# lambdaclass/simpleworks

Measured on AMD Instinct MI355X. Metric: Marlin prove() constraints/sec at 2^20 R1CS; G1 MSM points/sec, higher is better.
Workload: dtype u32 limbs (384-bit Montgomery Fq for G1, 256-bit Fr); 1 GPU; marlin_prove: synthetic R1CS, 2^20 constraints = variables = non-zeros per matrix (|H| = |K| = 2^20), SRS + proving key device resident; per_gpu_units=1048576, multi_gpu=replicas (one proof per rank)

## Files before the change

include/swmarlin.h:

```cpp
#ifndef SWMARLIN_H
#define SWMARLIN_H
#include <stddef.h>
#include <stdint.h>
#ifdef __cplusplus
extern "C" {
#endif

#define SWM_OK 0
#define SWM_ERR_INVALID_ARG (-1)
#define SWM_ERR_NO_DEVICE (-2)
#define SWM_ERR_HIP (-3)
#define SWM_ERR_OOM (-4)
#define SWM_ERR_UNSATISFIED (-5)
#define SWM_ERR_INDEX_TOO_LARGE (-6)
#define SWM_ERR_SERIALIZATION (-7)
#define SWM_ERR_MISMATCH (-8)
#define SWM_ERR_INTERNAL (-9)

typedef struct swm_ctx swm_ctx;
typedef struct swm_bases swm_bases;

int swm_version(void);
const char *swm_strerror(int code);
int swm_init(int device, swm_ctx **out);
void swm_destroy(swm_ctx *ctx);
const char *swm_last_error(swm_ctx *ctx);
int swm_set_stream(swm_ctx *ctx, void *hip_stream);
int swm_synchronize(swm_ctx *ctx);
int swm_malloc(swm_ctx *ctx, size_t bytes, void **dptr);
int swm_free(swm_ctx *ctx, void *dptr);
int swm_memcpy_h2d(swm_ctx *ctx, void *dst_dev, const void *src_host, size_t bytes);
int swm_memcpy_d2h(swm_ctx *ctx, void *dst_host, const void *src_dev, size_t bytes);

int swm_srs_upload(swm_ctx *ctx, const uint64_t *xy, size_t n, swm_bases **out);
int swm_srs_free(swm_ctx *ctx, swm_bases *bases);
size_t swm_srs_len(const swm_bases *bases);
int swm_msm_g1(swm_ctx *ctx, const swm_bases *bases, size_t offset, const uint64_t *scalars, size_t n,
               uint64_t out_jac[18]);
int swm_msm_g1_dev(swm_ctx *ctx, const swm_bases *bases, size_t offset, const void *d_scalars, size_t n,
                   int scalars_montgomery, uint64_t out_jac[18]);
int swm_g1_normalize(const uint64_t jac[18], uint64_t out_xy[12], int *is_inf);
int swm_g1_add_jac(const uint64_t a[18], const uint64_t b[18], uint64_t out[18]);

int swm_ntt_fr(swm_ctx *ctx, uint64_t *data, unsigned log_n, int inverse, int coset);
int swm_ntt_fr_dev(swm_ctx *ctx, void *d_data, unsigned log_n, int inverse, int coset);
int swm_ntt_fr_sharded_dev(swm_ctx *ctx, void *d_local, unsigned log_n, int inverse, int blocks_in);

int swm_spmv_fr(swm_ctx *ctx, const uint32_t *rowptr, const uint32_t *col, const uint64_t *val, const uint64_t *z,
                size_t z_len, uint64_t *out, size_t rows, size_t nnz);
int swm_spmv_fr_dev(swm_ctx *ctx, const void *d_rowptr, const void *d_col, const void *d_val, const void *d_z,
                    void *d_out, size_t rows);

int swm_batch_inverse_fr(swm_ctx *ctx, uint64_t *data, size_t n);
int swm_batch_inverse_fr_dev(swm_ctx *ctx, void *d_data, size_t n);
int swm_vec_mul_fr(swm_ctx *ctx, const uint64_t *a, const uint64_t *b, uint64_t *out, size_t n);
int swm_vec_mul_fr_dev(swm_ctx *ctx, const void *d_a, const void *d_b, void *d_out, size_t n);

typedef struct swm_rng swm_rng;
typedef struct swm_srs swm_srs;
typedef struct swm_pk swm_pk;
typedef struct swm_vk swm_vk;

int swm_rng_test_new(swm_rng **out);
int swm_rng_from_seed(const uint8_t seed[32], swm_rng **out);
typedef void (*swm_fill_bytes_fn)(void *user, uint8_t *dest, size_t len);
int swm_rng_from_callback(swm_fill_bytes_fn fill_bytes, void *user, swm_rng **out);
int swm_rng_from_chacha(const uint8_t key[32], uint64_t word_pos, int rounds, swm_rng **out);
int swm_rng_word_pos(const swm_rng *rng, uint64_t *word_pos);
int swm_rng_fill_bytes(swm_rng *rng, uint8_t *dest, size_t len);
void swm_rng_fill_bytes_cb(void *user, uint8_t *dest, size_t len);
void swm_rng_free(swm_rng *rng);
int swm_rng_next_u64(swm_rng *rng, uint64_t *out);
int swm_rng_rand_fr(swm_rng *rng, uint64_t out_mont[4]);

typedef struct swm_r1cs {
    size_t num_instance, num_witness, num_constraints;
    const uint64_t *instance;
    const uint64_t *witness;
    const uint32_t *a_rowptr, *a_col; const uint64_t *a_val;
    const uint32_t *b_rowptr, *b_col; const uint64_t *b_val;
// ... 369 lines not shown
```

simpleworks_amd/_lib.py:

```python
import contextlib
import ctypes
import json
import os

import numpy as np

_HERE = os.path.dirname(os.path.abspath(__file__))
LIB_PATH = os.environ.get("SWM_LIB_PATH") or os.path.join(_HERE, "libswmarlin.so")

_u64p = ctypes.POINTER(ctypes.c_uint64)
_u32p = ctypes.POINTER(ctypes.c_uint32)
_vp = ctypes.c_void_p
_sz = ctypes.c_size_t
_int = ctypes.c_int

ABI = {
    "swm_version": (_int, []),
    "swm_strerror": (ctypes.c_char_p, [_int]),
    "swm_init": (_int, [_int, ctypes.POINTER(_vp)]),
    "swm_destroy": (None, [_vp]),
    "swm_last_error": (ctypes.c_char_p, [_vp]),
    "swm_set_stream": (_int, [_vp, _vp]),
    "swm_set_msm_sharding": (_int, [_vp, ctypes.c_uint, ctypes.c_uint, _vp, _vp]),
    "swm_rccl_unique_id": (_int, [ctypes.c_void_p]),
    "swm_rccl_init": (_int, [_vp, ctypes.c_void_p, ctypes.c_uint, ctypes.c_uint]),
    "swm_set_rccl_comm": (_int, [_vp, _vp, ctypes.c_uint, ctypes.c_uint]),
    "swm_selftest_exchange": (_int, [_vp, ctypes.c_void_p, ctypes.c_void_p, _sz, _int]),
    "swm_rccl_info": (_int, [ctypes.c_char_p, _sz]),
    "swm_exchange_stats": (_int, [_vp, ctypes.POINTER(ctypes.c_uint64), ctypes.POINTER(ctypes.c_uint64)]),
    "swm_synchronize": (_int, [_vp]),
    "swm_malloc": (_int, [_vp, _sz, ctypes.POINTER(_vp)]),
    "swm_free": (_int, [_vp, _vp]),
    "swm_memcpy_h2d": (_int, [_vp, _vp, _vp, _sz]),
    "swm_memcpy_d2h": (_int, [_vp, _vp, _vp, _sz]),
    "swm_srs_upload": (_int, [_vp, _u64p, _sz, ctypes.POINTER(_vp)]),
    "swm_srs_free": (_int, [_vp, _vp]),
    "swm_srs_len": (_sz, [_vp]),
    "swm_msm_g1": (_int, [_vp, _vp, _sz, _u64p, _sz, _u64p]),
    "swm_msm_g1_dev": (_int, [_vp, _vp, _sz, _vp, _sz, _int, _u64p]),
    "swm_g1_normalize": (_int, [_u64p, _u64p, ctypes.POINTER(_int)]),
    "swm_g1_add_jac": (_int, [_u64p, _u64p, _u64p]),
    "swm_ntt_fr": (_int, [_vp, _u64p, ctypes.c_uint, _int, _int]),
    "swm_ntt_fr_dev": (_int, [_vp, _vp, ctypes.c_uint, _int, _int]),
    "swm_ntt_fr_sharded_dev": (_int, [_vp, ctypes.c_void_p, ctypes.c_uint, _int, _int]),
    "swm_spmv_fr": (_int, [_vp, _u32p, _u32p, _u64p, _u64p, _sz, _u64p, _sz, _sz]),
    "swm_spmv_fr_dev": (_int, [_vp, _vp, _vp, _vp, _vp, _vp, _sz]),
    "swm_batch_inverse_fr": (_int, [_vp, _u64p, _sz]),
    "swm_batch_inverse_fr_dev": (_int, [_vp, _vp, _sz]),
    "swm_vec_mul_fr": (_int, [_vp, _u64p, _u64p, _u64p, _sz]),
    "swm_vec_mul_fr_dev": (_int, [_vp, _vp, _vp, _vp, _sz]),
    "swm_rng_test_new": (_int, [ctypes.POINTER(_vp)]),
    "swm_rng_from_seed": (_int, [ctypes.c_void_p, ctypes.POINTER(_vp)]),
    "swm_rng_from_callback": (_int, [_vp, _vp, ctypes.POINTER(_vp)]),
    "swm_rng_from_chacha": (_int, [ctypes.c_void_p, ctypes.c_uint64, _int, ctypes.POINTER(_vp)]),
    "swm_rng_word_pos": (_int, [_vp, ctypes.POINTER(ctypes.c_uint64)]),
    "swm_rng_fill_bytes": (_int, [_vp, ctypes.c_void_p, ctypes.c_size_t]),
    "swm_rng_fill_bytes_cb": (None, [_vp, ctypes.c_void_p, ctypes.c_size_t]),
    "swm_rng_free": (None, [_vp]),
    "swm_rng_next_u64": (_int, [_vp, ctypes.POINTER(ctypes.c_uint64)]),
    "swm_rng_rand_fr": (_int, [_vp, _u64p]),
    "swm_generate_universal_srs": (_int, [_vp, _sz, _sz, _sz, _vp, ctypes.POINTER(_vp)]),
    "swm_srs_destroy": (None, [_vp, _vp]),
    "swm_srs_max_degree": (_sz, [_vp]),
    "swm_srs_power_of_g": (_int, [_vp, _vp, _sz, _u64p]),
    "swm_srs_export": (_int, [_vp, _vp, _sz, _sz, _u64p, _u64p, _u64p, _u64p]),
    "swm_srs_import": (_int, [_vp, _u64p, _sz, _u64p, _u64p, _u64p, ctypes.POINTER(_vp)]),
    "swm_generate_proving_and_verifying_keys": (_int, [_vp, _vp, ctypes.c_void_p, ctypes.POINTER(_vp), ctypes.POINTER(_vp)]),
    "swm_pk_destroy": (None, [_vp, _vp]),
    "swm_pk_retain": (_int, [_vp]),
    "swm_pk_attach": (_int, [_vp, _vp]),
    "swm_pk_device": (_int, [_vp]),
    "swm_pk_refcount": (_int, [_vp]),
    "swm_device_mem_info": (_int, [_vp, ctypes.POINTER(_sz), ctypes.POINTER(_sz)]),
    "swm_vk_destroy": (None, [_vp]),
    "swm_generate_proof": (_int, [_vp, _vp, ctypes.c_void_p, _vp, ctypes.c_void_p, _sz, ctypes.POINTER(_sz)]),
# ... 268 lines not shown
        return self

    def download(self, shape, dtype=np.uint64):
        out = np.empty(shape, dtype=dtype)
        assert out.nbytes <= self.nbytes
        self.ctx._check(self.ctx.lib.swm_memcpy_d2h(self.ctx.h, out.ctypes.data, self.ptr, out.nbytes), "swm_memcpy_d2h")
        return out

    def free(self):
        if self.ptr:
            self.ctx.lib.swm_free(self.ctx.h, self.ptr)
            self.ptr = None


class Bases:
    def __init__(self, ctx, handle, n):
        self.ctx, self.h, self.n = ctx, handle, n

    def free(self):
        if self.h:
            self.ctx.lib.swm_srs_free(self.ctx.h, self.h)
            self.h = None


class Context:

    def __init__(self, device=0):
        self.lib = load_library()
        h = _vp()
        rc = self.lib.swm_init(device, ctypes.byref(h))
        if rc != 0:
            raise SwmError(rc, "swm_init")
        self.h = h
        self.device = device

    def close(self):
        if self.h:
            self.lib.swm_destroy(self.h)
            self.h = None

    def __del__(self):
        try:
            self.close()
        except Exception:
            pass

    def _check(self, rc, what):
        if rc != 0:
            raise SwmError(rc, what, self.lib.swm_last_error(self.h).decode(errors="replace"))

    def set_stream(self, stream_ptr):
        self._check(self.lib.swm_set_stream(self.h, stream_ptr), "swm_set_stream")

    def synchronize(self):
        self._check(self.lib.swm_synchronize(self.h), "swm_synchronize")

    def mem_info(self):
        free, total = ctypes.c_size_t(0), ctypes.c_size_t(0)
        self._check(self.lib.swm_device_mem_info(self.h, ctypes.byref(free), ctypes.byref(total)), "swm_device_mem_info")
        return free.value, total.value

    ALLGATHER_FN = ctypes.CFUNCTYPE(ctypes.c_int, ctypes.c_void_p, ctypes.c_void_p, ctypes.c_size_t, ctypes.c_void_p)

    def set_msm_sharding(self, rank, world, allgather=None):
        if world <= 1 or allgather is None:
            self._check(self.lib.swm_set_msm_sharding(self.h, 0, 1, None, None), "swm_set_msm_sharding")
            self._shard_cb = None
            self.shard_rank, self.shard_world = 0, 1
            return
        self.shard_rank, self.shard_world = rank, world

        def _cb(_user, send, nbytes, recv):
            try:
                out = allgather(ctypes.string_at(send, nbytes))
                if len(out) != nbytes * world:
                    return 1
                ctypes.memmove(recv, out, len(out))
                return 0
            except Exception:
                import traceback
                traceback.print_exc()
                return 1
        cb = Context.ALLGATHER_FN(_cb)
        self._check(self.lib.swm_set_msm_sharding(self.h, rank, world, ctypes.cast(cb, ctypes.c_void_p), None),
                    "swm_set_msm_sharding")
        self._shard_cb = cb

    def rccl_init(self, unique_id, rank, world):
        buf = (ctypes.c_uint8 * 128).from_buffer_copy(bytes(unique_id))
        self._check(self.lib.swm_rccl_init(self.h, buf, rank, world), "swm_rccl_init")

    def selftest_exchange(self, send_buf, recv_buf, bytes_per_peer, alltoall=True):
        self._check(self.lib.swm_selftest_exchange(self.h, send_buf.ptr, recv_buf.ptr, bytes_per_peer, int(alltoall)), "swm_selftest_exchange")

    def exchange_stats(self):
        calls, nbytes = ctypes.c_uint64(0), ctypes.c_uint64(0)
        self._check(self.lib.swm_exchange_stats(self.h, ctypes.byref(calls), ctypes.byref(nbytes)), "swm_exchange_stats")
        return calls.value, nbytes.value

    def alloc(self, nbytes):
        return DeviceBuffer(self, nbytes)

    def to_device(self, arr):
        arr = np.ascontiguousarray(arr)
        return DeviceBuffer(self, max(arr.nbytes, 64)).upload(arr)

# ... 902 lines not shown
```

simpleworks_amd/csrc/capi.hip:

```cpp
#include <dlfcn.h>
#include <stdarg.h>
#include <string.h>
#include <algorithm>
#include <vector>
#include "context.h"
#include "g1.cuh"
#include "msm.h"

struct swm_rccl_id_arg {
    char internal[128];
};

namespace swm {

int ntt_run(swm_ctx* ctx, void* d_data, unsigned log_n, int inverse, int coset);
int ntt_sharded_run(swm_ctx* ctx, void* d_local, unsigned log_n, int inverse, int blocks_in);
struct SpmvPlan;
int spmv_run(swm_ctx* ctx, const void* d_rowptr, const void* d_col, const void* d_val, const void* d_z, void* d_out,
             size_t rows, const SpmvPlan* plan = nullptr);
int vec_mul_run(swm_ctx* ctx, const void* a, const void* b, void* out, size_t n);
int batch_inverse_run(swm_ctx* ctx, void* d, size_t n);
int selftest_mul_run(swm_ctx* ctx, int which, const void* a, const void* b, void* out, size_t n);
int selftest_chain_run(swm_ctx* ctx, int which, void* out, size_t threads, int iters);
int selftest_g1_add_run(swm_ctx* ctx, const void* a, const void* b, void* out, size_t n);
// ... 466 lines not shown
    if (!rccl().ok) return rccl_unavailable(ctx);
    rccl_release(ctx);
    swm_rccl_id_arg arg;
    memcpy(arg.internal, id, 128);
    void* comm = nullptr;
    int rc = rccl().CommInitRank(&comm, (int)world, arg, (int)rank);
    if (rc != 0) return rccl_fail(ctx, "ncclCommInitRank", rc);
    ctx->rccl_comm = comm;
    ctx->rccl_own = true;
    ctx->shard_rank = rank;
    ctx->shard_world = world;
    ctx->shard_allgather = nullptr;
    ctx->shard_user = nullptr;
    return SWM_OK;
}
int swm_set_rccl_comm(swm_ctx* ctx, void* nccl_comm, unsigned rank, unsigned world) {
    if (!ctx) return SWM_ERR_INVALID_ARG;
    rccl_release(ctx);
    if (!nccl_comm) {
        ctx->shard_rank = 0;
        ctx->shard_world = 1;
        return SWM_OK;
    }
    if (world == 0 || rank >= world) return SWM_ERR_INVALID_ARG;
    if (!rccl().ok) return rccl_unavailable(ctx);
    ctx->rccl_comm = nccl_comm;
    ctx->rccl_own = false;
    ctx->shard_rank = rank;
    ctx->shard_world = world;
    ctx->shard_allgather = nullptr;
    ctx->shard_user = nullptr;
    return SWM_OK;
}
int swm_rccl_info(char* buf, size_t cap) {
    if (!buf || cap == 0) return SWM_ERR_INVALID_ARG;
    const std::string d = rccl_describe();
    snprintf(buf, cap, "%s", d.c_str());
    return rccl().ok ? SWM_OK : SWM_ERR_INTERNAL;
}
int swm_exchange_stats(swm_ctx* ctx, uint64_t* calls, uint64_t* bytes_per_rank) {
    if (!ctx) return SWM_ERR_INVALID_ARG;
    if (calls) *calls = ctx->stat_exchanges;
    if (bytes_per_rank) *bytes_per_rank = ctx->stat_exchange_bytes;
    return SWM_OK;
}

int swm_set_stream(swm_ctx* ctx, void* hip_stream) {
    if (!ctx) return SWM_ERR_INVALID_ARG;
    SWM_ON_DEVICE(ctx);
    SWM_HIP(ctx, hipStreamSynchronize(ctx->stream));
    ctx->stream = hip_stream ? (hipStream_t)hip_stream : ctx->own_stream;
    return SWM_OK;
}
int swm_synchronize(swm_ctx* ctx) {
    if (!ctx) return SWM_ERR_INVALID_ARG;
    SWM_ON_DEVICE(ctx);
    SWM_HIP(ctx, hipStreamSynchronize(ctx->stream));
    return SWM_OK;
}
int swm_malloc(swm_ctx* ctx, size_t bytes, void** dptr) {
    if (!ctx || !dptr) return SWM_ERR_INVALID_ARG;
    SWM_ON_DEVICE(ctx);
    SWM_HIP(ctx, hipMalloc(dptr, bytes ? bytes : 1));
    return SWM_OK;
}
int swm_free(swm_ctx* ctx, void* dptr) {
    if (!ctx) return SWM_ERR_INVALID_ARG;
    SWM_ON_DEVICE(ctx);
    SWM_HIP(ctx, hipStreamSynchronize(ctx->stream));
    SWM_HIP(ctx, hipFree(dptr));
    return SWM_OK;
}
int swm_memcpy_h2d(swm_ctx* ctx, void* dst, const void* src, size_t bytes) {
    if (!ctx) return SWM_ERR_INVALID_ARG;
    SWM_ON_DEVICE(ctx);
    SWM_HIP(ctx, hipMemcpyAsync(dst, src, bytes, hipMemcpyHostToDevice, ctx->stream));
    SWM_HIP(ctx, hipStreamSynchronize(ctx->stream));
    return SWM_OK;
}
int swm_memcpy_d2h(swm_ctx* ctx, void* dst, const void* src, size_t bytes) {
    if (!ctx) return SWM_ERR_INVALID_ARG;
    SWM_ON_DEVICE(ctx);
    SWM_HIP(ctx, hipMemcpyAsync(dst, src, bytes, hipMemcpyDeviceToHost, ctx->stream));
    SWM_HIP(ctx, hipStreamSynchronize(ctx->stream));
    return SWM_OK;
}

int swm_srs_upload(swm_ctx* ctx, const uint64_t* xy, size_t n, swm_bases** out) {
    if (!ctx || !xy || !out || n == 0) return set_err(ctx, SWM_ERR_INVALID_ARG, "srs_upload: bad arguments");
    SWM_ON_DEVICE(ctx);
    swm_bases* b = new swm_bases();
    b->n = n;
    hipError_t e = hipMalloc(&b->d_points, n * sizeof(G1Affine));
    if (e != hipSuccess) {
        delete b;
        return set_err(ctx, SWM_ERR_OOM, "srs_upload: %s", hipGetErrorString(e));
    }
    e = hipMemcpyAsync(b->d_points, xy, n * sizeof(G1Affine), hipMemcpyHostToDevice, ctx->stream);
    if (e == hipSuccess) e = hipStreamSynchronize(ctx->stream);
    if (e != hipSuccess) {
        (void)hipFree(b->d_points);
        delete b;
        return set_err(ctx, SWM_ERR_HIP, "srs_upload: %s", hipGetErrorString(e));
    }
    const size_t mask_words = (n + 31) / 32;
    int rc = SWM_OK;
// ... 436 lines not shown
```

simpleworks_amd/csrc/context.h:

```cpp
#pragma once
#include <hip/hip_runtime.h>
#include <stdint.h>
#include <stdio.h>
#include <map>
#include <string>
#include <vector>
#include "../../include/swmarlin.h"
#include "host/pool.h"
#include "host/witness_chunks.h"
#include "switches.h"

namespace swm {

struct MsmJob;
struct DevBuf {
    void* p = nullptr;
    size_t cap = 0;
};

struct NttTables {
    void* lo = nullptr;
    void* hi = nullptr;
    size_t hi_len = 0;
};
// ... 20 lines not shown
    size_t ntt_pass_table_bytes = 0;
    static constexpr int MSM_SLOTS = 8;
    static constexpr int MSM_LANES = 4;
    hipStream_t aux_stream[MSM_LANES] = {nullptr, nullptr, nullptr, nullptr};
    std::vector<hipStream_t> spare_streams;
    hipEvent_t fork_event = nullptr;
    void* pinned = nullptr;
    void* pinned_dev = nullptr;
    void* h2d_stage = nullptr;
    size_t h2d_stage_used = 0;
    const void* witness_dev = nullptr;
    size_t witness_stage_bytes = swm::WITNESS_STAGE_BYTES;
    hipEvent_t slot_event[MSM_SLOTS] = {nullptr};
    bool slot_busy[MSM_SLOTS] = {false};
    hipEvent_t acc_event[MSM_SLOTS] = {nullptr};
    hipEvent_t sort_event[MSM_SLOTS] = {nullptr};
    hipEvent_t set_acc_event[4] = {nullptr, nullptr, nullptr, nullptr};
    hipEvent_t lane_copy_event[4] = {nullptr, nullptr, nullptr, nullptr};
    hipEvent_t twin_sorted_event = nullptr;
    hipEvent_t twin_copy_event[MSM_SLOTS] = {nullptr};
    std::vector<swm::MsmJob*> pending_tails;
    swm::MsmJob* lazy_tail = nullptr;
    int next_slot = 0;
    std::multimap<size_t, void*> pool;
    uint64_t stat_msm_digits = 0;
    uint64_t stat_msm_twins = 0;
    uint64_t stat_msm_adds = 0;
    uint64_t stat_msm_zero_points = 0;
    uint64_t stat_spmv_nnz = 0;
    std::vector<std::pair<char, uint64_t>> call_log;
    void log_call(char kind, uint64_t v) {
        if (profiling && call_log.size() < 8192) call_log.push_back({kind, v});
    }
    uint64_t stat_msm_calls = 0, stat_msm_points = 0, stat_ntt_calls = 0, stat_ntt_elems = 0, stat_spmv_calls = 0,
             stat_spmv_rows = 0;
    int profiling = 0;
    bool prof_open = false;
    std::map<std::string, swm::ProfAgg> prof;
    std::vector<swm::ProfPending> pending;
    std::vector<hipEvent_t> event_pool;
    unsigned shard_rank = 0, shard_world = 1;
    swm_allgather_fn shard_allgather = nullptr;
    void* shard_user = nullptr;
    void* rccl_comm = nullptr;
    bool rccl_own = false;
    void *rccl_send = nullptr, *rccl_recv = nullptr;
    size_t rccl_cap = 0;
    uint64_t stat_exchanges = 0, stat_exchange_bytes = 0;
    swm::HostPool* host_pool = nullptr;
    hipStream_t copy_stream = nullptr;
    void* ext_pinned = nullptr;
    bool ext_registered = false;
    size_t msm_pipe_min = 0;
    size_t msm_slot_bytes[6] = {0, 0, 0, 0, 0, 0};
    bool emulated_exchange = false;
    unsigned msm_since_wait = 0;
    uint32_t* ext_totals = nullptr;
    hipEvent_t ext_cnt_event[8] = {nullptr, nullptr, nullptr, nullptr, nullptr, nullptr, nullptr, nullptr};
    hipEvent_t ext_event[5] = {nullptr, nullptr, nullptr, nullptr, nullptr};
};

struct swm_bases {
    void* d_points = nullptr;
    void* d_points28 = nullptr;
    uint32_t* d_inf_mask = nullptr;
    unsigned table_c = 0;
    void* d_te = nullptr;
    size_t n = 0;
};

namespace swm {

int set_err(swm_ctx* ctx, int code, const char* fmt, ...);
void drain_streams(swm_ctx* ctx);
int shard_exchange(swm_ctx* ctx, const void* send, size_t bytes, void* recv);
int shard_allgather_dev(swm_ctx* ctx, const void* d_send, size_t bytes, void* d_recv);
int shard_alltoall_dev(swm_ctx* ctx, const void* d_send, void* d_recv, size_t bytes_per_peer);

struct DeviceGuard {
    int prev = -1;
    bool ok = true, switched = false;
    explicit DeviceGuard(const swm_ctx* ctx) {
        if (!ctx) return;
        if (hipGetDevice(&prev) != hipSuccess) prev = -1;
        if (prev != ctx->device) {
            ok = hipSetDevice(ctx->device) == hipSuccess;
            switched = ok && prev >= 0;
        }
    }
    ~DeviceGuard() {
        if (switched) (void)hipSetDevice(prev);
    }
};
#define SWM_ON_DEVICE(ctx)                                                                             \
    swm::DeviceGuard dev_guard__(ctx);                                                                 \
    if (!dev_guard__.ok) return swm::set_err(ctx, SWM_ERR_HIP, "hipSetDevice(%d) failed", (ctx)->device)
int scratch(swm_ctx* ctx, const char* name, size_t bytes, void** out);
void scratch_release(swm_ctx* ctx, const char* name);
int pool_alloc(swm_ctx* ctx, size_t bytes, void** out, size_t* cap);
void pool_free(swm_ctx* ctx, void* p, size_t cap);
int get_root_tables(swm_ctx* ctx, unsigned log_n, int inverse, NttTables** out);
void prof_begin(swm_ctx* ctx, const char* name);
void prof_end(swm_ctx* ctx);
void prof_flush(swm_ctx* ctx);

#define SWM_HIP(ctx, call)                                                                              \
// ... 23 lines not shown
```

simpleworks_amd/csrc/marlin.hip:

```cpp
#include <stdlib.h>
#include <string.h>
#include <algorithm>
#include <chrono>
#include <functional>
#include <memory>
#include <type_traits>
#include "devops.cuh"
#include "g1.cuh"
#include "host/ahp.h"

#include "msm.h"
using namespace swm;

#define LAUNCHX(ctx, name, kernel, grid, block, shmem, ...)                         \
    do {                                                                            \
        prof_begin(ctx, name);                                                      \
        hipLaunchKernelGGL(kernel, grid, block, shmem, (ctx)->stream, __VA_ARGS__); \
        prof_end(ctx);                                                              \
        hip_check(ctx, hipGetLastError(), name);                                    \
    } while (0)

#include "host/pk_codec.h"
#include "host/host_handles.h"
struct swm_srs {
// ... 992 lines not shown
    __device__ __forceinline__ Fr at(size_t i) const {
        const unsigned q = (unsigned)(i & 3);
        return q == 0 ? n0 : q == 1 ? n1 : q == 2 ? n2 : n3;
    }
};
RAlphaNumerators r_alpha_numerators(const Fr& alpha, unsigned logH, uint64_t M) {
    Fr aH = alpha;
    for (unsigned i = 0; i < logH; i++) aH = fp_sqr(aH);
    Fr i4 = HDomain(M).gen;
    for (unsigned i = 0; i < logH; i++) i4 = fp_sqr(i4);
    return {fp_sub(aH, fp_one<Fr>()), fp_sub(aH, i4), fp_sub(aH, fp_sqr(i4)), fp_sub(aH, fp_mul(fp_sqr(i4), i4))};
}
struct DenseMap {
    __host__ __device__ size_t index(size_t p) const { return p; }
};
struct BlocksMap {
    size_t loc, blk, rank;
    __host__ __device__ size_t index(size_t p) const { return loc * (p / blk) + rank * blk + (p % blk); }
};
struct CosetsMap {
    unsigned logD;
    __host__ __device__ size_t index(size_t p) const { return ((p & (((size_t)1 << logD) - 1)) << 2) + (p >> logD); }
    __host__ __device__ size_t position(size_t i) const { return ((i & 3) << logD) + (i >> 2); }
};
template <class F>
void with_product_map(const ShardPlan& sp, bool sharded, size_t loc, bool cosets, unsigned logD, F&& f) {
    if (sharded) f(BlocksMap{loc, loc / sp.SG, sp.rank});
    else if (cosets) f(CosetsMap{logD});
    else f(DenseMap{});
}
__device__ __forceinline__ Fr round2_outer_form(const Fr& eta_a, const Fr& eta_b, const Fr& eta_c, const Fr& ra, const Fr& a,
                                                const Fr& b, const Fr& z, const Fr& t) {
    const Fr summed = fp_add(fp_add(fp_mul(eta_c, fp_mul(a, b)), fp_mul(eta_a, a)), fp_mul(eta_b, b));
    return fp_sub(fp_mul(ra, summed), fp_mul(z, t));
}
struct IndexOnB {
    const Fr *ar, *ac, *arc, *av;
    const Fr *br, *bc, *brc, *bv;
    const Fr *cr, *cc, *crc, *cv;
};
struct Round3Challenges {
    Fr alpha, beta, ab, ve_a, ve_b, ve_c;
};
__device__ __forceinline__ Fr round3_a_minus_bf(const IndexOnB& x, const Round3Challenges& c, size_t i, const Fr& f) {
    Fr da = fp_add(fp_sub(fp_sub(c.ab, fp_mul(x.ar[i], c.alpha)), fp_mul(c.beta, x.ac[i])), x.arc[i]);
    Fr db = fp_add(fp_sub(fp_sub(c.ab, fp_mul(x.br[i], c.alpha)), fp_mul(c.beta, x.bc[i])), x.brc[i]);
    Fr dc = fp_add(fp_sub(fp_sub(c.ab, fp_mul(x.cr[i], c.alpha)), fp_mul(c.beta, x.cc[i])), x.crc[i]);
    Fr dbc = fp_mul(db, dc);
    Fr ua = fp_mul(c.ve_a, x.av[i]), ub = fp_mul(c.ve_b, x.bv[i]), uc = fp_mul(c.ve_c, x.cv[i]);
    Fr a_val = fp_add(fp_mul(ua, dbc), fp_mul(da, fp_add(fp_mul(ub, dc), fp_mul(uc, db))));
    Fr b_val = fp_mul(da, dbc);
    return fp_sub(a_val, fp_mul(b_val, f));
}
struct ProveState {
    ChaChaRng& zk;
    PhaseTrace& tr;
    const ProveShape shape;
    const ShardPlan sp;
    const uint64_t H, K, X, Bsz, M;
    const unsigned logM;
    const size_t nvars, ninst;
    const size_t mask_len;
    const HDomain dh;
    const std::vector<Fr> public_input;
    FiatShamirRng fs;
    VerifierState st;
    Fr rho_w, rho_a, rho_b;
    int lane = 0;
    LPoly P_w, P_za, P_zb, P_mask, P_t, P_g1, P_h1, P_g2, P_h2;
    LPoly idx_polys[12];
    std::map<std::string, LPoly*> polys;
    CommitJob j1[4], j2[3], j3[2];
    std::vector<Commitment> comms1 = std::vector<Commitment>(4), comms2 = std::vector<Commitment>(3),
                            comms3 = std::vector<Commitment>(2);
    bool mask_late = false;
    unsigned mask_pieces = 1;
    AsyncMsm mask_part[2];
    bool ra_closed_form = false;
    bool cosets = false;
    LcSet lcs;
    DVec mask, z, za_evals, zb_evals, za_loc, zb_loc, x_poly, w_poly, za_poly, zb_poly, e_za, e_zb, e_z;
    DVec r_alpha_evals, e_ra, t_poly, q1, h1, g1x, f, h2;

    ProveState(const swm_pk& pk, ChaChaRng& rng, PhaseTrace& t, ProveShape shp, const ShardPlan& plan)
        : zk(rng), tr(t), shape(std::move(shp)), sp(plan), H(pk.H), K(pk.K), X(pk.X), Bsz(pk.B), M(4 * pk.H),
          logM(pk.logH + 2), nvars(pk.info.num_variables), ninst(shape.inst.size()), mask_len(3 * pk.H), dh(pk.H),
          public_input(shape.inst.begin() + 1, shape.inst.end()) {
        fs_init(fs, pk.vk, public_input);
        for (int m = 0; m < 3; m++) {
            const DVec* v[4] = {&pk.ar[m].row, &pk.ar[m].col, &pk.ar[m].val, &pk.ar[m].row_col};
            for (int j = 0; j < 4; j++) {
                idx_polys[4 * m + j].p = v[j]->p;
                idx_polys[4 * m + j].n = K;
                polys[kIndexerPolys[4 * m + j]] = &idx_polys[4 * m + j];
            }
        }
        polys["w"] = &P_w; polys["z_a"] = &P_za; polys["z_b"] = &P_zb; polys["mask_poly"] = &P_mask;
        polys["t"] = &P_t; polys["g_1"] = &P_g1; polys["h_1"] = &P_h1; polys["g_2"] = &P_g2; polys["h_2"] = &P_h2;
    }
};

void draw_mask(swm_ctx* ctx, const swm_pk& pk, ProveState& s) {
    const uint64_t H = s.H;
    Fr* mp = s.mask.p;
    if (s.mask_pieces > 1) {
        CommitJob& job = s.j1[3];
        job.has_bound = false;
        job.hiding = false;
        unsigned done_pieces = 0;
        struct PieceEvent {
            hipEvent_t e = nullptr;
            ~PieceEvent() {
                if (e) (void)hipEventDestroy(e);
            }
        } piece_guard;
        hip_check(ctx, hipEventCreateWithFlags(&piece_guard.e, hipEventDisableTiming), "event");
        const hipEvent_t piece_ev = piece_guard.e;
        auto enqueue_piece = [&](unsigned pc) {
            hip_check(ctx, hipEventRecord(piece_ev, ctx->copy_stream), "record");
            hip_check(ctx, hipStreamWaitEvent(ctx->stream, piece_ev, 0), "wait");
            if (pc == 0) commit_enqueue(ctx, &s.lane, pk, 1, mp + 1, H - 1, &job.plain);
            else if (s.mask_pieces == 3) commit_enqueue(ctx, &s.lane, pk, pc * H, mp + pc * H, H, &s.mask_part[pc - 1]);
            else if (pc == 2) commit_enqueue(ctx, &s.lane, pk, H, mp + H, 2 * H, &s.mask_part[0]);
        };
        const std::function<void(size_t)> progress = [&](size_t have) {
            while (done_pieces < 2 && have >= (size_t)(done_pieces + 1) * H) enqueue_piece(done_pieces++);
        };
        sample_fr_bulk(ctx, s.zk, mp, s.mask_len, s.mask_late, &progress);
        while (done_pieces < 3) enqueue_piece(done_pieces++);
    } else {
        sample_fr_bulk(ctx, s.zk, mp, s.mask_len, s.mask_late);
    }
    ew(ctx, "mask_fix", 1, [=] __device__(size_t) {
        mp[0] = fp_neg(fp_add(mp[H], mp[2 * H]));
    });
// ... 385 lines not shown
            e_f = shard_evals(ctx, s.sp, s.f.p, K, pk.logB);
        } else if constexpr (cosets) {
            static const unsigned ks[3] = {1, 2, 3};
            e_f = DVec(ctx, 3 * K);
            rc_check(ctx, ntt_cosets_fwd(ctx, s.f.p, K, pk.logK, ks, 3, e_f.p));
        } else {
            e_f = dv_ntt_from(ctx, s.f.p, K, pk.logB, false);
        }
        DVec ab(ctx, Bloc);
        Fr* out = ab.p;
        const bool on_K_every_4th = Bsz == 4 * K;
        const Fr* pf = e_f.p;
        ew(ctx, "round3_pointwise_B", Bloc, [=] __device__(size_t p) {
            if constexpr (cosets) {
                out[p] = (p & 3) == 0 ? fp_zero<Fr>() : round3_a_minus_bf(ix, ch, p, pf[map.position(p) - K]);
            } else {
                const size_t i = map.index(p);
                out[p] = on_K_every_4th && (i & 3) == 0 ? fp_zero<Fr>() : round3_a_minus_bf(ix, ch, i, pf[p]);
            }
        });
        if constexpr (blocks) {
            const size_t Kl = K / s.sp.SG;
            rc_check(ctx, ntt_sharded_run(ctx, ab.p, pk.logB, 1, 1));
            DVec loc(ctx, 3 * Kl);
            div_vk(ctx, ab.p, Kl, Bloc, loc.p);
            shard_gather_cyclic(ctx, loc.p, 3 * Kl, s.sp.slog_g, s.h2.p, 3 * K);
        } else {
            dv_ntt(ctx, ab, pk.logB, true);
            div_vk(ctx, ab.p, K, Bsz, s.h2.p);
        }
    });
    s.P_h2.p = s.h2.p;
    s.P_h2.n = 3 * K >= 3 ? 3 * K - 3 : 0;
}

std::vector<Fr> evaluations(swm_ctx* ctx, const swm_pk& pk, ProveState& s) {
    std::map<std::pair<std::string, bool>, Fr> eval_cache;
    {
        std::vector<std::pair<std::string, bool>> want;
        for (const char* l : {"z_b", "t", "g_1", "mask_poly", "z_a", "w", "h_1"}) want.push_back({l, false});
        for (int i = 0; i < 12; i++) want.push_back({kIndexerPolys[i], true});
        want.push_back({"g_2", true});
        want.push_back({"h_2", true});
        DVec slots(ctx, want.size());
        auto enqueue_at = [&](bool at_gamma, const EvalPoint& ep) {
            std::vector<EvalItem> items;
            for (size_t i = 0; i < want.size(); i++) {
                if (want[i].second != at_gamma) continue;
                LPoly* lp = s.polys.at(want[i].first);
                items.push_back({lp->p, lp->n, slots.p + i});
            }
            poly_eval_many(ctx, items, ep);
        };
        EvalPoint ep_beta = eval_point(ctx, s.st.beta);
        enqueue_at(false, ep_beta);
        commit_gather(ctx, {&s.j3[0].plain, &s.j3[0].shifted, &s.j3[1].plain});
        pc_commit_end_round(ctx, pk, {&s.j3[0], &s.j3[1]}, {nullptr, nullptr}, {&s.P_g2.rand, &s.P_h2.rand}, s.comms3.data());
        s.tr.mark("round 3 commitments");
        fs_absorb_commitments(s.fs, s.comms3);
        s.st.gamma = s.fs.rand_fr();
        EvalPoint ep_gamma = eval_point(ctx, s.st.gamma);
        enqueue_at(true, ep_gamma);
        std::vector<Fr> vals = slots.download(0, want.size());
        for (size_t i = 0; i < want.size(); i++) eval_cache[want[i]] = vals[i];
    }
    const Fr beta = s.st.beta, gamma = s.st.gamma;
    auto poly_at = [&](const std::string& label, const Fr& point) {
        bool at_gamma = fp_eq(point, gamma);
        auto key = std::make_pair(label, at_gamma);
        auto it = eval_cache.find(key);
        if (it != eval_cache.end()) return it->second;
        LPoly* lp = s.polys.at(label);
        Fr v = poly_eval(ctx, lp->p, lp->n, point);
        eval_cache[key] = v;
        return v;
    };
    auto provider = [&](const std::string&, const LcTerms& terms, const Fr& point) {
        Fr acc = fp_zero<Fr>();
        for (auto& t : terms) acc = fp_add(acc, t.second.empty() ? t.first : fp_mul(t.first, poly_at(t.second, point)));
        return acc;
    };
    s.lcs = construct_linear_combinations(pk.info, s.public_input, provider, s.st);
    std::vector<std::pair<std::string, Fr>> evals;
    for (auto& q : kQuerySet) {
        const Fr& pt = std::string(q.point) == "beta" ? beta : gamma;
        Fr v = provider(q.label, s.lcs.at(q.label), pt);
        if (lc_has_zero_eval(q.label)) {
            if (!fp_is_zero(v) && !ctx->emulated_exchange)
                throw MarlinError(SWM_ERR_UNSATISFIED, std::string(q.label) + " does not evaluate to zero: constraint system is not satisfied");
            continue;
        }
        evals.push_back({q.label, v});
    }
    std::sort(evals.begin(), evals.end(), [](auto& a, auto& b) { return a.first < b.first; });
    std::vector<Fr> out;
    for (auto& e : evals) out.push_back(e.second);
    return out;
}

#ifndef SWM_OPEN_FOLD
#define SWM_OPEN_FOLD 1
#endif
__global__ void __launch_bounds__(256) open_fold_shifted(Fr* __restrict__ wq, const Fr* __restrict__ sq, size_t n, Fr k) {
    SWM_LIGHT_KERNEL();
    for (size_t t = blockIdx.x * (size_t)blockDim.x + threadIdx.x; t < n; t += (size_t)gridDim.x * blockDim.x)
        wq[t] = fp_add(wq[t], fp_mul(sq[t], k));
}
std::vector<PcProof> open_combinations(swm_ctx* ctx, const swm_pk& pk, ProveState& s, const Fr& xi) {
    struct ShiftedTerm {
        LPoly* lp;
        Fr ch;
    };
    static constexpr int MAX_COMBINE = 24;
    struct CombineTerms {
        const Fr* src[MAX_COMBINE];
        size_t len[MAX_COMBINE];
        Fr k[MAX_COMBINE];
    };
    struct PointOpen {
        Fr point;
        DivResult wq;
        std::vector<DivResult> sq;
        AsyncMsm wjob;
        std::vector<AsyncMsm> sjobs;
        AsyncMsm folded_slot;
        bool folded = false;
        HPoly r_comb, shifted_r, shifted_r_witness;
        std::vector<ShiftedTerm> shifted_terms;
    };
    const char* points[2] = {"beta", "gamma"};
    PointOpen po[2];
    for (int pi = 0; pi < 2; pi++) {
        const char* pl = points[pi];
        PointOpen& o = po[pi];
        o.point = pi == 0 ? s.st.beta : s.st.gamma;
        const Fr point = o.point;
        std::vector<std::string> labels;
        for (auto& q : kQuerySet)
            if (std::string(q.point) == pl) labels.push_back(q.label);
        std::sort(labels.begin(), labels.end());
        size_t plen = 0;
        for (auto& l : labels)
            for (auto& t : s.lcs.at(l))
                if (!t.second.empty()) plen = std::max(plen, s.polys.at(t.second)->n);
        CombineTerms cterms;
        int nterms = 0;
        Fr ch = fr_one();
        for (auto& l : labels) {
            const LcTerms& terms = s.lcs.at(l);
            bool single_bounded = false;
            for (auto& t : terms) {
                if (t.second.empty()) continue;
                LPoly* lp = s.polys.at(t.second);
                if (terms.size() == 1 && lp->has_bound) single_bounded = true;
                else if (lp->has_bound) throw MarlinError(SWM_ERR_INTERNAL, "EquationHasDegreeBounds");
                Fr k = fp_mul(ch, t.first);
                if (nterms >= MAX_COMBINE) throw MarlinError(SWM_ERR_INTERNAL, "too many terms in an opening");
                cterms.src[nterms] = lp->p;
                cterms.len[nterms] = lp->n;
                cterms.k[nterms] = k;
                nterms++;
                hp_add_scaled(o.r_comb, lp->rand.rand, k);
            }
            ch = fp_mul(ch, xi);
            if (single_bounded) {
                LPoly* lp = s.polys.at(terms[0].second);
                o.shifted_terms.push_back({lp, ch});
                hp_add_scaled(o.shifted_r, lp->rand.shifted_rand, ch);
                if (!hp_is_zero(lp->rand.shifted_rand)) hp_add_scaled(o.shifted_r_witness, hp_div_linear(lp->rand.shifted_rand, point), ch);
                ch = fp_mul(ch, xi);
            }
        }
        size_t wn = plen ? plen - 1 : 0;
        std::vector<bool> folded(o.shifted_terms.size(), false);
        for (size_t i = 0; i < o.shifted_terms.size(); i++) {
            const LPoly* lp = o.shifted_terms[i].lp;
            const size_t off = pk.srs_max_degree - lp->bound, qn = lp->n ? lp->n - 1 : 0;
            folded[i] = SWM_OPEN_FOLD && qn && pk.in_powers(off, qn);
            if (folded[i]) wn = std::max(wn, off + qn);
        }
        {
            DVec work(ctx, std::max<size_t>(plen, wn + 1));
            Fr* out = work.p;
            const int nt = nterms;
            ew(ctx, "open_combine", work.n, [=] __device__(size_t i) {
                Fr acc = fp_zero<Fr>();
                for (int j = 0; j < nt; j++)
                    if (i < cterms.len[j]) acc = fp_add(acc, fp_mul(cterms.k[j], cterms.src[j][i]));
                out[i] = acc;
            });
            s.tr.tick(pi == 0 ? "open beta: combination enqueued" : "open gamma: combination enqueued");
            o.wq = div_linear_in_place(ctx, std::move(work), plen, point);
        }
        s.tr.tick("  witness quotient enqueued");
        const bool fold_any = std::find(folded.begin(), folded.end(), true) != folded.end();
        if (!fold_any) {
            commit_enqueue(ctx, &s.lane, pk, 0, o.wq.work.p + 1, wn, &o.wjob);
            s.tr.tick("  witness commitment enqueued");
        }
        o.sq.resize(o.shifted_terms.size());
        o.sjobs.reserve(o.shifted_terms.size());
        for (size_t i = 0; i < o.shifted_terms.size(); i++) {
            auto& stt = o.shifted_terms[i];
            o.sq[i] = div_linear(ctx, stt.lp->p, stt.lp->n, point);
            Fr k = stt.ch;
            Fr* q = o.sq[i].work.p;
            const size_t off = pk.srs_max_degree - stt.lp->bound, qn = stt.lp->n ? stt.lp->n - 1 : 0;
            if (folded[i]) {
                const unsigned grid = (unsigned)std::min<size_t>((qn + 255) / 256, 256 * 32);
                LAUNCHX(ctx, "open_fold_shifted", open_fold_shifted, dim3(grid), dim3(256), 0, o.wq.work.p + 1 + off, q + 1, qn, k);
                s.tr.tick("  shifted quotient folded");
                continue;
            }
            ew(ctx, "open_scale", qn, [=] __device__(size_t t) { q[t + 1] = fp_mul(q[t + 1], k); });
            s.tr.tick("  shifted quotient enqueued");
            o.sjobs.emplace_back();
            commit_enqueue(ctx, &s.lane, pk, off, q + 1, qn, &o.sjobs.back());
            s.tr.tick("  shifted commitment enqueued");
        }
        if (fold_any) {
            commit_enqueue(ctx, &s.lane, pk, 0, o.wq.work.p + 1, wn, &o.wjob);
            s.tr.tick("  witness commitment enqueued");
            o.folded = true;
            o.folded_slot.sharded = o.wjob.sharded;
            o.folded_slot.result = g1_xyzz_identity();
        }
    }
    commit_flush(ctx);
    s.tr.tick("open: bucket stages enqueued");
    G1XYZZ hide[2];
    std::vector<PcProof> pps(2);
    for (int pi = 0; pi < 2; pi++) {
        PointOpen& o = po[pi];
        hide[pi] = g1_xyzz_identity();
        if (!hp_is_zero(o.r_comb)) {
            g1_add(hide[pi], gamma_msm(pk, hp_div_linear(o.r_comb, o.point)));
            pps[pi].has_random_v = true;
            pps[pi].random_v = host_poly_eval(o.r_comb, o.point);
        }
        if (!o.shifted_terms.empty()) {
            if (!hp_is_zero(o.shifted_r_witness)) g1_add(hide[pi], gamma_msm(pk, o.shifted_r_witness));
            if (!hp_is_zero(o.shifted_r) && pps[pi].has_random_v)
                pps[pi].random_v = fp_add(pps[pi].random_v, host_poly_eval(o.shifted_r, o.point));
        }
    }
    auto second = [](PointOpen& o) { return !o.sjobs.empty() ? &o.sjobs[0] : o.folded ? &o.folded_slot : nullptr; };
    commit_gather(ctx, {&po[0].wjob, second(po[0]), &po[1].wjob, second(po[1])});
    G1XYZZ wit[2];
    G1Affine wit_aff[2];
    for (int pi = 0; pi < 2; pi++) {
        PointOpen& o = po[pi];
        wit[pi] = commit_wait(ctx, &o.wjob);
        for (AsyncMsm& sj : o.sjobs) g1_add(wit[pi], commit_wait(ctx, &sj));
        g1_add(wit[pi], hide[pi]);
    }
    g1_to_affine_batch(wit, 2, wit_aff);
    for (int pi = 0; pi < 2; pi++) pps[pi].w = wit_aff[pi];
    return pps;
}

std::vector<uint8_t> prove_impl(swm_ctx* ctx, const swm_pk& pk, const swm_r1cs* cs, ChaChaRng& zk, bool uncompressed = false) {
    PhaseTrace tr(ctx);
    if (sw(SW_TRACE) >= 1 || sw(SW_PROOF_MARKS)) hipLaunchKernelGGL(swm_proof_begin, dim3(1), dim3(1), 0, ctx->stream);
    ProveShape shape = prove_shape(cs, pk);
    tr.mark("pad_and_square");
    shard_agree(ctx, pk);
    ctx->emulated_exchange = false;
    ProveState s(pk, zk, tr, std::move(shape), shard_plan(ctx, pk));
    struct PipeMinScope {
        swm_ctx* c;
        ~PipeMinScope() { c->msm_pipe_min = 0; }
    } pipe_scope{ctx};
    ctx->msm_pipe_min = pk.logH <= (unsigned)sw(SW_PROVE_ONE_STREAM_LOG) ? ~(size_t)0 : 0;

    s.rho_w = zk.rand_fr();
    s.rho_a = zk.rand_fr();
    s.rho_b = zk.rand_fr();
    begin_mask(ctx, pk, s);
    upload_witness(ctx, pk, s, cs);
    tr.mark("upload z, z_A, z_B");
    round1_polys(ctx, pk, s);
    tr.mark("round 1 polynomials");
    if (!s.mask_late) commit_flush(ctx);
    round2_prework(ctx, s);
    if (s.mask_late) {
        draw_mask(ctx, pk, s);
        commit_flush(ctx);
    }
    tr.tick("r1: pre-work enqueued");
    round1_commitments(ctx, pk, s);
    tr.mark("round 1 commitments");
    fs_absorb_commitments(s.fs, s.comms1);
    s.st.alpha = s.fs.sample_outside(s.dh);
    s.st.eta_a = s.fs.rand_fr();
    s.st.eta_b = s.fs.rand_fr();
    s.st.eta_c = s.fs.rand_fr();

    r_alpha(ctx, pk, s);
    round2_t(ctx, pk, s);
    round2_q1(ctx, pk, s);
    tr.mark("round 2 polynomials");
    round2_commitments(ctx, pk, s);
    tr.mark("round 2 commitments");
    fs_absorb_commitments(s.fs, s.comms2);
    s.st.beta = s.fs.sample_outside(s.dh);

    round3_polys(ctx, pk, s);
    tr.mark("round 3 polynomials");
    pc_commit_begin(ctx, pk, &s.lane, s.P_h2.p, s.P_h2.n, false, 0, false, &s.j3[1]);
    commit_flush(ctx);

    Proof proof;
    proof.evaluations = evaluations(ctx, pk, s);
    tr.mark("evaluations");
    fs_absorb_evals(s.fs, proof.evaluations);
    const Fr xi = s.fs.challenge_u128();
    proof.pc_proof = open_combinations(ctx, pk, s, xi);
    tr.mark("openings");
    proof.commitments = {s.comms1, s.comms2, s.comms3};
    return serialize_proof(proof, uncompressed);
}
// ... 727 lines not shown
```

Before: 23.14 million constraints/s.

## Compute beta evaluations via synthetic division and reuse quotients in opening

When opening at beta, each polynomial is divided by (X - beta) once, early in round 3. The evaluation is read from the division remainder slot, replacing the separate multi-point evaluation pass. The opening step then builds the witness quotient as a linear combination of these stored quotients instead of combining the polynomials and dividing again, and the shifted quotients are scaled from the same buffers. This drops one evaluation pass and the repeated divisions. In exchange it keeps the per-polynomial quotient buffers alive longer, adding memory pressure, and it only applies in the single-GPU case.

```diff
diff --git a/include/swmarlin.h b/include/swmarlin.h
--- a/include/swmarlin.h
+++ b/include/swmarlin.h
@@ -26,6 +26,7 @@
 void swm_destroy(swm_ctx *ctx);
 const char *swm_last_error(swm_ctx *ctx);
 int swm_set_stream(swm_ctx *ctx, void *hip_stream);
+int swm_set_prelude_early(swm_ctx *ctx, unsigned mask);
 int swm_synchronize(swm_ctx *ctx);
 int swm_malloc(swm_ctx *ctx, size_t bytes, void **dptr);
 int swm_free(swm_ctx *ctx, void *dptr);
diff --git a/simpleworks_amd/_lib.py b/simpleworks_amd/_lib.py
--- a/simpleworks_amd/_lib.py
+++ b/simpleworks_amd/_lib.py
@@ -21,6 +21,7 @@
     "swm_destroy": (None, [_vp]),
     "swm_last_error": (ctypes.c_char_p, [_vp]),
     "swm_set_stream": (_int, [_vp, _vp]),
+    "swm_set_prelude_early": (_int, [_vp, ctypes.c_uint]),
     "swm_set_msm_sharding": (_int, [_vp, ctypes.c_uint, ctypes.c_uint, _vp, _vp]),
     "swm_rccl_unique_id": (_int, [ctypes.c_void_p]),
     "swm_rccl_init": (_int, [_vp, ctypes.c_void_p, ctypes.c_uint, ctypes.c_uint]),
@@ -395,6 +396,9 @@
     def set_stream(self, stream_ptr):
         self._check(self.lib.swm_set_stream(self.h, stream_ptr), "swm_set_stream")
 
+    def set_prelude_early(self, mask):
+        self._check(self.lib.swm_set_prelude_early(self.h, mask), "swm_set_prelude_early")
+
     def synchronize(self):
         self._check(self.lib.swm_synchronize(self.h), "swm_synchronize")
 
diff --git a/simpleworks_amd/csrc/capi.hip b/simpleworks_amd/csrc/capi.hip
--- a/simpleworks_amd/csrc/capi.hip
+++ b/simpleworks_amd/csrc/capi.hip
@@ -542,6 +542,11 @@
     ctx->stream = hip_stream ? (hipStream_t)hip_stream : ctx->own_stream;
     return SWM_OK;
 }
+int swm_set_prelude_early(swm_ctx* ctx, unsigned mask) {
+    if (!ctx || mask > 1) return SWM_ERR_INVALID_ARG;
+    ctx->prelude_early = mask;
+    return SWM_OK;
+}
 int swm_synchronize(swm_ctx* ctx) {
     if (!ctx) return SWM_ERR_INVALID_ARG;
     SWM_ON_DEVICE(ctx);
diff --git a/simpleworks_amd/csrc/context.h b/simpleworks_amd/csrc/context.h
--- a/simpleworks_amd/csrc/context.h
+++ b/simpleworks_amd/csrc/context.h
@@ -96,6 +96,7 @@
     void* ext_pinned = nullptr;
     bool ext_registered = false;
     size_t msm_pipe_min = 0;
+    unsigned prelude_early = 1;
     size_t msm_slot_bytes[6] = {0, 0, 0, 0, 0, 0};
     bool emulated_exchange = false;
     unsigned msm_since_wait = 0;
diff --git a/simpleworks_amd/csrc/marlin.hip b/simpleworks_amd/csrc/marlin.hip
--- a/simpleworks_amd/csrc/marlin.hip
+++ b/simpleworks_amd/csrc/marlin.hip
@@ -1068,6 +1068,10 @@
     Fr b_val = fp_mul(da, dbc);
     return fp_sub(a_val, fp_mul(b_val, f));
 }
+#ifndef SWM_PRELUDE_EARLY
+#define SWM_PRELUDE_EARLY 1
+#endif
+enum : unsigned { PRELUDE_BETA_QUOT = 1 };
 struct ProveState {
     ChaChaRng& zk;
     PhaseTrace& tr;
@@ -1097,6 +1101,12 @@
     LcSet lcs;
     DVec mask, z, za_evals, zb_evals, za_loc, zb_loc, x_poly, w_poly, za_poly, zb_poly, e_za, e_zb, e_z;
     DVec r_alpha_evals, e_ra, t_poly, q1, h1, g1x, f, h2;
+    unsigned prelude = 0;
+    struct BetaQuotient {
+        const LPoly* lp;
+        DivResult q;
+    };
+    std::vector<BetaQuotient> beta_quot;
 
     ProveState(const swm_pk& pk, ChaChaRng& rng, PhaseTrace& t, ProveShape shp, const ShardPlan& plan)
         : zk(rng), tr(t), shape(std::move(shp)), sp(plan), H(pk.H), K(pk.K), X(pk.X), Bsz(pk.B), M(4 * pk.H),
@@ -1588,8 +1598,28 @@
             }
             poly_eval_many(ctx, items, ep);
         };
-        EvalPoint ep_beta = eval_point(ctx, s.st.beta);
-        enqueue_at(false, ep_beta);
+        EvalPoint ep_beta;
+        if ((s.prelude & PRELUDE_BETA_QUOT) && ctx->shard_world <= 1) {
+            static constexpr int MAX_AT_BETA = 8;
+            struct Heads {
+                const Fr* src[MAX_AT_BETA];
+                Fr* dst[MAX_AT_BETA];
+            } heads;
+            size_t nh = 0;
+            for (size_t i = 0; i < want.size(); i++) {
+                if (want[i].second) continue;
+                if (nh >= MAX_AT_BETA) throw MarlinError(SWM_ERR_INTERNAL, "too many polynomials at beta");
+                const LPoly* lp = s.polys.at(want[i].first);
+                s.beta_quot.push_back({lp, div_linear(ctx, lp->p, lp->n, s.st.beta)});
+                heads.src[nh] = s.beta_quot.back().q.work.p;
+                heads.dst[nh] = slots.p + i;
+                nh++;
+            }
+            ew(ctx, "beta_values", nh, [=] __device__(size_t j) { *heads.dst[j] = *heads.src[j]; });
+        } else {
+            ep_beta = eval_point(ctx, s.st.beta);
+            enqueue_at(false, ep_beta);
+        }
         commit_gather(ctx, {&s.j3[0].plain, &s.j3[0].shifted, &s.j3[1].plain});
         pc_commit_end_round(ctx, pk, {&s.j3[0], &s.j3[1]}, {nullptr, nullptr}, {&s.P_g2.rand, &s.P_h2.rand}, s.comms3.data());
         s.tr.mark("round 3 commitments");
@@ -1651,6 +1681,11 @@
     struct CombineTerms {
         const Fr* src[MAX_COMBINE];
         size_t len[MAX_COMBINE];
+        Fr k[MAX_COMBINE];
+    };
+    struct QuotientTerms {
+        const Fr* src[MAX_COMBINE];
+        size_t len[MAX_COMBINE], off[MAX_COMBINE];
         Fr k[MAX_COMBINE];
     };
     struct PointOpen {
@@ -1680,6 +1715,7 @@
             for (auto& t : s.lcs.at(l))
                 if (!t.second.empty()) plen = std::max(plen, s.polys.at(t.second)->n);
         CombineTerms cterms;
+        const LPoly* cpoly[MAX_COMBINE];
         int nterms = 0;
         Fr ch = fr_one();
         for (auto& l : labels) {
@@ -1695,6 +1731,7 @@
                 cterms.src[nterms] = lp->p;
                 cterms.len[nterms] = lp->n;
                 cterms.k[nterms] = k;
+                cpoly[nterms] = lp;
                 nterms++;
                 hp_add_scaled(o.r_comb, lp->rand.rand, k);
             }
@@ -1715,7 +1752,45 @@
             folded[i] = SWM_OPEN_FOLD && qn && pk.in_powers(off, qn);
             if (folded[i]) wn = std::max(wn, off + qn);
         }
-        {
+        const bool from_quotients = pi == 0 && !s.beta_quot.empty();
+        auto quotient_of = [&](const LPoly* lp) -> const Fr* {
+            for (auto& bq : s.beta_quot)
+                if (bq.lp == lp) return bq.q.work.p;
+            throw MarlinError(SWM_ERR_INTERNAL, "an opening at beta of a polynomial that was not divided");
+        };
+        if (from_quotients) {
+            QuotientTerms qt;
+            int nq = 0;
+            auto add_term = [&](const Fr* src, size_t len, size_t off, const Fr& k) {
+                if (!len) return;
+                for (int j = 0; j < nq; j++)
+                    if (qt.src[j] == src && qt.off[j] == off) {
+                        qt.k[j] = fp_add(qt.k[j], k);
+                        return;
+                    }
+                if (nq >= MAX_COMBINE) throw MarlinError(SWM_ERR_INTERNAL, "too many terms in an opening");
+                qt.src[nq] = src;
+                qt.len[nq] = len;
+                qt.off[nq] = off;
+                qt.k[nq] = k;
+                nq++;
+            };
+            for (int j = 0; j < nterms; j++)
+                add_term(quotient_of(cpoly[j]) + 1, cterms.len[j] ? cterms.len[j] - 1 : 0, 0, cterms.k[j]);
+            for (size_t i = 0; i < o.shifted_terms.size(); i++) {
+                const LPoly* lp = o.shifted_terms[i].lp;
+                if (folded[i]) add_term(quotient_of(lp) + 1, lp->n - 1, pk.srs_max_degree - lp->bound, o.shifted_terms[i].ch);
+            }
+            o.wq.work = DVec(ctx, wn + 1);
+            Fr* out = o.wq.work.p + 1;
+            ew(ctx, "open_combine_quotients", wn, [=] __device__(size_t i) {
+                Fr acc = fp_zero<Fr>();
+                for (int j = 0; j < nq; j++)
+                    if (i >= qt.off[j] && i - qt.off[j] < qt.len[j]) acc = fp_add(acc, fp_mul(qt.k[j], qt.src[j][i - qt.off[j]]));
+                out[i] = acc;
+            });
+            s.tr.tick("open beta: witness combined from the quotients");
+        } else {
             DVec work(ctx, std::max<size_t>(plen, wn + 1));
             Fr* out = work.p;
             const int nt = nterms;
@@ -1738,17 +1813,26 @@
         o.sjobs.reserve(o.shifted_terms.size());
         for (size_t i = 0; i < o.shifted_terms.size(); i++) {
             auto& stt = o.shifted_terms[i];
-            o.sq[i] = div_linear(ctx, stt.lp->p, stt.lp->n, point);
+            const size_t off = pk.srs_max_degree - stt.lp->bound, qn = stt.lp->n ? stt.lp->n - 1 : 0;
             Fr k = stt.ch;
-            Fr* q = o.sq[i].work.p;
-            const size_t off = pk.srs_max_degree - stt.lp->bound, qn = stt.lp->n ? stt.lp->n - 1 : 0;
-            if (folded[i]) {
-                const unsigned grid = (unsigned)std::min<size_t>((qn + 255) / 256, 256 * 32);
-                LAUNCHX(ctx, "open_fold_shifted", open_fold_shifted, dim3(grid), dim3(256), 0, o.wq.work.p + 1 + off, q + 1, qn, k);
-                s.tr.tick("  shifted quotient folded");
-                continue;
+            Fr* q;
+            if (from_quotients) {
+                if (folded[i]) continue;
+                o.sq[i].work = DVec(ctx, qn + 1);
+                q = o.sq[i].work.p;
+                const Fr* src = quotient_of(stt.lp);
+                ew(ctx, "open_scale", qn, [=] __device__(size_t t) { q[t + 1] = fp_mul(src[t + 1], k); });
+            } else {
+                o.sq[i] = div_linear(ctx, stt.lp->p, stt.lp->n, point);
+                q = o.sq[i].work.p;
+                if (folded[i]) {
+                    const unsigned grid = (unsigned)std::min<size_t>((qn + 255) / 256, 256 * 32);
+                    LAUNCHX(ctx, "open_fold_shifted", open_fold_shifted, dim3(grid), dim3(256), 0, o.wq.work.p + 1 + off, q + 1, qn, k);
+                    s.tr.tick("  shifted quotient folded");
+                    continue;
+                }
+                ew(ctx, "open_scale", qn, [=] __device__(size_t t) { q[t + 1] = fp_mul(q[t + 1], k); });
             }
-            ew(ctx, "open_scale", qn, [=] __device__(size_t t) { q[t + 1] = fp_mul(q[t + 1], k); });
             s.tr.tick("  shifted quotient enqueued");
             o.sjobs.emplace_back();
             commit_enqueue(ctx, &s.lane, pk, off, q + 1, qn, &o.sjobs.back());
@@ -1803,6 +1887,7 @@
     shard_agree(ctx, pk);
     ctx->emulated_exchange = false;
     ProveState s(pk, zk, tr, std::move(shape), shard_plan(ctx, pk));
+    s.prelude = ctx->prelude_early & SWM_PRELUDE_EARLY;
     struct PipeMinScope {
         swm_ctx* c;
         ~PipeMinScope() { c->msm_pipe_min = 0; }
```

New measurement: 23.26 million constraints/s, median of 6. No clear change (+0.5%).
